# LivGen/LMAT

Hardware: AMD Instinct MI355X
Metric: reads/s (150 bp) vs 64 GB k-mer DB (higher is better)
Workload: dtype u64; 1 GPU; 1104000000 x 150 bp reads/GPU vs 64 GiB k-mer hash (6467472668 20-mers, replicated per GPU), run_rl.sh flags -x 0 -j 30 -l 0 -b 1, calls-only; total_reads=1104000000, reads_per_launch=8000000, read_len=150, db_kmers=6467472668, k=20, parallelism=reads sharded x1, DB replicated, genus_block_permille=100, prune_g=0, list_replicas=1, distinct_lists=792576, reads_called=1058323347, read_pool_batches=32

## Files before the change

### lmat_amd/csrc/kernels.hip

```cpp
#include <hip/hip_runtime.h>
#include <atomic>
#include <type_traits>
#include "kernels.hpp"

#ifndef LMAT_ABLATE
#define LMAT_ABLATE 0
#endif
#define STOP_AT(n, v) do { if (LMAT_ABLATE && A.prm.stop_after == (n)) { if (lane == 0) { emit(250, (v)); } return; } } while (0)
#ifndef LMAT_CLOSURE_FAST
#define LMAT_CLOSURE_FAST 1
#endif
#ifndef LMAT_LIST_INLINE
#define LMAT_LIST_INLINE 1
#endif
#ifndef LMAT_EVEN_K
#define LMAT_EVEN_K 3
#endif
#ifndef LMAT_LDS_SHIFT
#define LMAT_LDS_SHIFT 0
#endif

namespace lmat {

#define WSYNC()                                              \
    do {                                                     \
        __builtin_amdgcn_fence(__ATOMIC_SEQ_CST, "wavefront"); \
        __builtin_amdgcn_wave_barrier();                     \
    } while (0)

template <bool GMEM>
__device__ __forceinline__ void wsync() {
    if (GMEM) __builtin_amdgcn_fence(__ATOMIC_SEQ_CST, "workgroup");
    else __builtin_amdgcn_fence(__ATOMIC_SEQ_CST, "wavefront");
    __builtin_amdgcn_wave_barrier();
}
static const int kGmemU = 32768;
static const int kGmemGrid = 2048;

#define GAS __attribute__((address_space(1)))
typedef uint32_t u32x4 __attribute__((ext_vector_type(4)));
typedef uint32_t u32x4_a4 __attribute__((ext_vector_type(4), aligned(4)));
typedef unsigned short u16x2 __attribute__((ext_vector_type(2)));
typedef uint32_t u32x2 __attribute__((ext_vector_type(2)));
#define LAS __attribute__((address_space(3)))
#define G_ADD(p, v) __hip_atomic_fetch_add((p), (v), __ATOMIC_RELAXED, __HIP_MEMORY_SCOPE_AGENT)
#define G_OR(p, v) __hip_atomic_fetch_or((p), (v), __ATOMIC_RELAXED, __HIP_MEMORY_SCOPE_AGENT)
__device__ __forceinline__ void store_result(GAS uint64_t* dst, const lmat_read_result& r) {
    static_assert(sizeof(lmat_read_result) == 40, "result record is 5 x 8 bytes");
    uint64_t w[5];
    __builtin_memcpy(w, &r, 40);
    dst[0] = w[0]; dst[1] = w[1]; dst[2] = w[2]; dst[3] = w[3]; dst[4] = w[4];
}

__device__ __forceinline__ uint64_t lt_mask(int lane) { return lane == 0 ? 0ull : (~0ull >> (64 - lane)); }
__device__ __forceinline__ int popc64(uint64_t x) { return __popcll(x); }
__device__ __forceinline__ uint32_t wave_scan_incl(uint32_t x) {
    x += (uint32_t)__builtin_amdgcn_update_dpp(0, (int)x, 0x111, 0xf, 0xf, true);
    x += (uint32_t)__builtin_amdgcn_update_dpp(0, (int)x, 0x112, 0xf, 0xf, true);
    x += (uint32_t)__builtin_amdgcn_update_dpp(0, (int)x, 0x114, 0xf, 0xf, true);
    x += (uint32_t)__builtin_amdgcn_update_dpp(0, (int)x, 0x118, 0xf, 0xf, true);
    x += (uint32_t)__builtin_amdgcn_update_dpp(0, (int)x, 0x142, 0xa, 0xf, false);
    x += (uint32_t)__builtin_amdgcn_update_dpp(0, (int)x, 0x143, 0xc, 0xf, false);
    return x;
}
__device__ __forceinline__ uint32_t wave_scan_max(uint32_t x) {
    x = max(x, (uint32_t)__builtin_amdgcn_update_dpp(0, (int)x, 0x111, 0xf, 0xf, true));
    x = max(x, (uint32_t)__builtin_amdgcn_update_dpp(0, (int)x, 0x112, 0xf, 0xf, true));
    x = max(x, (uint32_t)__builtin_amdgcn_update_dpp(0, (int)x, 0x114, 0xf, 0xf, true));
    x = max(x, (uint32_t)__builtin_amdgcn_update_dpp(0, (int)x, 0x118, 0xf, 0xf, true));
    x = max(x, (uint32_t)__builtin_amdgcn_update_dpp(0, (int)x, 0x142, 0xa, 0xf, false));
    x = max(x, (uint32_t)__builtin_amdgcn_update_dpp(0, (int)x, 0x143, 0xc, 0xf, false));
    return x;
}
__device__ __forceinline__ uint32_t wave_sum(uint32_t x) { return (uint32_t)__builtin_amdgcn_readlane((int)wave_scan_incl(x), 63); }
__device__ __forceinline__ uint32_t prefix_count(uint64_t m) {
    return __builtin_amdgcn_mbcnt_hi((uint32_t)(m >> 32), __builtin_amdgcn_mbcnt_lo((uint32_t)m, 0u));
}
__device__ __forceinline__ bool lane_bit(uint64_t m) { return __builtin_amdgcn_inverse_ballot_w64(m); }
__device__ __forceinline__ uint32_t hash32(uint64_t x) {
    x *= 0x9E3779B97F4A7C15ull;
    return (uint32_t)(x >> 40);
}

__device__ __forceinline__ uint32_t zero_bytes(uint32_t z) {
    const uint32_t t = (z & 0x7F7F7F7Fu) + 0x7F7F7F7Fu;
    return ~(t | z | 0x7F7F7F7Fu);
}
__global__ __launch_bounds__(256) void pack_reads_kernel(const uint8_t* __restrict__ bases,
                                                         const uint64_t* __restrict__ off,
                                                         const uint64_t* __restrict__ rec_off,
                                                         uint32_t* __restrict__ words, uint64_t n) {
    const int lane = threadIdx.x & 63;
    const uint32_t sub = (uint32_t)lane & 15u;
    const uint64_t wave = (uint64_t)blockIdx.x * (blockDim.x >> 6) + (threadIdx.x >> 6);
    const uint64_t nw = (uint64_t)gridDim.x * (blockDim.x >> 6);
    for (uint64_t r0 = wave * 4; r0 < n; r0 += nw * 4) {
        const uint64_t r = r0 + ((uint32_t)lane >> 4);
        const bool have = r < n;
        const uint64_t b0 = have ? off[r] : 0;
        const uint32_t len = have ? (uint32_t)(off[r + 1] - b0) : 0u;
        uint32_t* rec = words + (have ? rec_off[r] : 0);
        if (have && sub == 0) rec[0] = len;
        const uint32_t nb = (len + 15) / 16;
        for (uint32_t p0 = 0; __ballot(p0 < len) != 0; p0 += 256) {
            const uint32_t p = p0 + 16u * sub;
            uint32_t code = 0, valid16 = 0;
            if (p < len) {
                const uint64_t addr = b0 + p, a4 = addr & ~3ull, end = b0 + len;
                const uint32_t sh = (uint32_t)(addr & 3) * 8u;
                const uint32_t* src = (const uint32_t*)(bases + a4);
                uint32_t d[5];
#pragma unroll
                for (int q = 0; q < 5; ++q) d[q] = a4 + 4u * q < end ? src[q] : 0u;
                const uint32_t left = len - p;
#pragma unroll
                for (int q = 0; q < 4; ++q) {
                    uint32_t w = __builtin_amdgcn_alignbit(d[q + 1], d[q], sh);
                    if (left < 4u * q + 4u) w &= left > 4u * q ? (1u << (8u * (left - 4u * q))) - 1u : 0u;
                    const uint32_t x = w & 0xDFDFDFDFu;
                    const uint32_t vm = zero_bytes(x ^ 0x41414141u) | zero_bytes(x ^ 0x43434343u) | zero_bytes(x ^ 0x47474747u) | zero_bytes(x ^ 0x54545454u);
                    const uint32_t v1 = vm >> 7;
                    const uint32_t c2 = (((x >> 1) & 0x03030303u) ^ ((x >> 2) & 0x01010101u)) & (v1 * 3u);
                    code |= ((c2 | (c2 >> 6) | (c2 >> 12) | (c2 >> 18)) & 0xFFu) << (8 * q);
                    valid16 |= ((v1 | (v1 >> 7) | (v1 >> 14) | (v1 >> 21)) & 0xFu) << (4 * q);
                }
                if ((p >> 4) < nb) rec[1 + (p >> 4)] = code;
            }
            const uint32_t other = (uint32_t)__shfl_xor((int)valid16, 1);
            if (p < len && (sub & 1u) == 0) rec[1 + nb + (p >> 5)] = valid16 | (other << 16);
        }
    }
}

__device__ __forceinline__ bool wide_insert(uint64_t* slots, uint32_t nbuckets, uint32_t b, uint64_t kmer, uint32_t payload) {
    const uint64_t val = (kmer << kPayloadBits) | payload;
    const uint32_t max_tries = nbuckets < (1u << 14) ? nbuckets : (1u << 14);
    for (uint32_t tries = 0; tries < max_tries; ++tries) {
        unsigned long long* s = (unsigned long long*)(slots + (uint64_t)b * kSlotsPerBucket);
        for (int j = 0; j < kSlotsPerBucket; ++j) {
            unsigned long long old = s[j];
            while (true) {
                if (old == 0) {
                    unsigned long long prev = atomicCAS(&s[j], 0ull, (unsigned long long)val);
                    if (prev == 0) return true;
                    old = prev;
                    continue;
                }
                if ((old >> kPayloadBits) == kmer) {
                    if (old <= val) return true;
                    unsigned long long prev = atomicCAS(&s[j], old, (unsigned long long)val);
                    if (prev == old) return true;
                    old = prev;
                    continue;
                }
                break;
            }
        }
        b = b + 1 == nbuckets ? 0 : b + 1;
    }
    return false;
}
__device__ __forceinline__ uint32_t wide_lookup(const uint64_t* __restrict__ slots, uint32_t nbuckets, uint32_t b, uint64_t kmer) {
    for (uint32_t tries = 0; tries < nbuckets; ++tries) {
        const uint64_t* s = slots + (uint64_t)b * kSlotsPerBucket;
        bool empty = false;
        for (int j = 0; j < kSlotsPerBucket; ++j) {
            const uint64_t v = s[j];
            if (v == 0) empty = true;
            else if ((v >> kPayloadBits) == kmer) return (uint32_t)(v & kPayloadMask);
// ... 221 lines not shown
        const uint32_t nb = (len + 15) / 16;
        for (uint32_t w0 = 0; w0 < nb; w0 += 64) {
            const uint32_t w = w0 + lane;
            uint32_t code = 0, valid = 0;
            if (w < nb) {
                for (int j = 0; j < 16; ++j) {
                    const uint32_t p = w * 16 + j;
                    if (p >= len) break;
                    uint32_t b;
                    if (kind < 10) {
                        b = (uint32_t)(splitmix(h0 ^ ((uint64_t)p << 20) ^ 0x1234567) >> 9) & 3u;
                    } else if (kind == 10) {
                        b = (uint32_t)(splitmix(h0 ^ ((uint64_t)(p % 25) << 20) ^ 0x7654321) >> 9) & 3u;
                    } else {
                        const uint64_t gp = rc ? goff + (len - 1 - p) : goff + p;
                        b = synth_strain_base(g, sp, sg, gp < G ? gp : G - 1);
                        if (rc) b ^= 3u;
                        const uint64_t e = splitmix(h0 ^ ((uint64_t)p << 24) ^ 0xABCDEF);
                        if ((e % 100) == 0) b = (b + 1 + (uint32_t)((e >> 32) % 3)) & 3u;
                    }
                    bool ok = !(kind == 11 && p == npos);
                    code |= (ok ? b : 0u) << (2 * j);
                    valid |= (ok ? 1u : 0u) << j;
                }
                rec[1 + w] = code;
            }
            uint32_t other = __shfl_down(valid, 1);
            if (w < nb && (w & 1) == 0) rec[1 + nb + (w >> 1)] = valid | (((w + 1 < nb) ? other : 0u) << 16);
        }
    }
}

__global__ void lookup_kernel(DeviceTables tb, const uint64_t* __restrict__ kmers, uint64_t n, uint32_t* counts,
                              uint32_t* tids, uint32_t stride) {
    uint64_t i = (uint64_t)blockIdx.x * blockDim.x + threadIdx.x;
    if (i >= n) return;
    const uint32_t pay = table_lookup(tb, kmers[i]);
    if (pay == 0) { counts[i] = 0; return; }
    if (pay < kListBase) {
        counts[i] = 1;
        if (stride) tids[i * stride] = tb.tid32[pay];
        return;
    }
    const size_t eoff = LMAT_LIST_OFF(pay, tb.list_shift);
    if (tb.arena[eoff] & 0x8000u) {
        const uint32_t n = tb.arena[eoff + 1];
        counts[i] = n;
        for (uint32_t j = 0; j < n && j < stride; ++j)
            tids[i * stride + j] = (uint32_t)tb.arena[eoff + kListHdr + 2 * j] | ((uint32_t)tb.arena[eoff + kListHdr + 2 * j + 1] << 16);
        return;
    }
    const uint32_t nk = tb.arena[eoff + 1], nr = tb.arena[eoff + 2];
    counts[i] = nr;
    if (tb.wide) {
        const size_t raw = eoff + kListHdr + 4 * (size_t)nk;
        for (uint32_t j = 0; j < nr && j < stride; ++j) tids[i * stride + j] = (uint32_t)tb.arena[raw + 2 * j] | ((uint32_t)tb.arena[raw + 2 * j + 1] << 16);
        return;
    }
    for (uint32_t j = 0; j < nr && j < stride; ++j) tids[i * stride + j] = tb.conv[tb.arena[eoff + kListHdr + 2 * nk + j]];
}

__global__ void probe_stats_kernel(DeviceTables tb, const uint64_t* __restrict__ kmers, uint64_t n, unsigned long long* out) {
    const uint64_t i = (uint64_t)blockIdx.x * blockDim.x + threadIdx.x;
    if (i >= n || !tb.cpt.nb) return;
    const uint64_t kmer = kmers[i], rc = revcomp_fwd(kmer, tb.cpt.k);
    uint32_t b, tag;
    cpt_address(tb.cpt, kmer < rc ? kmer : rc, kmer < rc ? rc : kmer, b, tag);
    const uint32_t* bk = (const uint32_t*)tb.slots + (uint64_t)b * 16;
    if (kmer <= rc)
        for (int j = 0; j < kCptSlots; ++j)
            if (((const uint16_t*)bk)[j] == (uint16_t)tag) { atomicAdd(&out[0], 1ull); return; }
    if (!(bk[15] & kCptOvfFlag)) { atomicAdd(&out[1], 1ull); return; }
    uint32_t ob = ovf_bucket_of(b, tag, tb.ovf_nbuckets);
    unsigned long long reads = 0;
    for (uint32_t tries = 0; tries < tb.ovf_nbuckets; ++tries) {
        const uint64_t* s_ = tb.ovf_slots + (uint64_t)ob * kSlotsPerBucket;
        ++reads;
        bool empty = false;
        for (int j = 0; j < kSlotsPerBucket; ++j) {
            const uint64_t v = s_[j];
            if (v == 0) empty = true;
            else if ((v >> kPayloadBits) == kmer) { atomicAdd(&out[2], 1ull); atomicAdd(&out[4], reads); return; }
        }
        if (empty) break;
        ob = ob + 1 == tb.ovf_nbuckets ? 0 : ob + 1;
    }
    atomicAdd(&out[3], 1ull);
    atomicAdd(&out[4], reads);
}

struct LinEnt {
    uint16_t tid;
    uint16_t dep;
    uint16_t tin, tout;
    float score;
};
static const uint16_t kLinNoGood = 0x8000;
struct LinEntW {
    uint32_t tid;
    uint16_t dep, pad_;
    uint32_t tin, tout;
    float score;
};
static const int kFastE = 256;
static const int kK4SmallT = 16;
static const int kK4MidT = 32;
template <int TT> struct K4Lds {
    static constexpr int LIN = TT + (TT <= 16 ? 3 : 8);
    static constexpr int LANES = TT <= 32 ? 64 : 32;
    static constexpr int STRIDE = ((17 * TT + 12 * LIN + 3) / 4) | 1;
    static constexpr int BYTES = STRIDE * 4 * LANES;
    static_assert(8 * TT <= 12 * LIN, "sort keys over the lineage entries");
};
static_assert(K4Lds<16>::STRIDE == 125, "small tier: 31.25 KB per wave");

constexpr int pow2_ceil(int x) { int p = 1; while (p < x) p <<= 1; return p; }

template <int U, int T, int E, bool INK4, bool CPT = false, bool WIDE = false>
struct WL {
    static constexpr int IDB = WIDE ? 4 : 2;
    static constexpr int HB = WIDE ? 8 : 4;
    static_assert(!WIDE || INK4, "wide ids run in the classes that keep their tables in memory and decide in-kernel");
    static constexpr int H = pow2_ceil(U * 3 / 2);
    static constexpr int D = INK4 ? U : 64;
    static constexpr int TH = 4 * T;
    static constexpr int LIN = T + 72;
    static constexpr int RD_WORDS = (U + 96) / 16 + (U + 96) / 32 + 4;
    static constexpr int R1_HASH = 8 * H;
    static constexpr int R1_TID = (IDB + 6) * T + 2 * HB * TH + (INK4 ? (4 + 2 * IDB) * T + 4 * T + T + 4 * T + 4 * T + T : 0);
    static constexpr bool HASH_OVER = CPT && U <= 512 && !INK4;
    static constexpr int R1 = HASH_OVER ? R1_TID : (R1_HASH > R1_TID ? R1_HASH : R1_TID);
    static constexpr int R2_K = CPT ? 0 : 8 * U + 4 * U;
    static constexpr int R2_D = 4 * D + 2 * D + 2 * D + 2 * D + D;
    static constexpr int R2_L = INK4 ? (WIDE ? 20 : 12) * LIN : 0;
    static constexpr int R2 = R2_K > R2_D ? (R2_K > R2_L ? R2_K : R2_L) : (R2_D > R2_L ? R2_D : R2_L);
    static constexpr int R3_P = 4 * U;
    static constexpr int R3_E = (INK4 ? (WIDE ? 24 : 16) : 7) * E;
    static constexpr int R3 = R3_P > R3_E ? R3_P : R3_E;
    static constexpr int OFF_RD = 0;
    static constexpr int OFF_R1 = CPT && U <= 512 ? 0 : ((RD_WORDS * 4 + 15) / 16) * 16;
    static constexpr int OFF_R2 = OFF_R1 + ((R1 + 15) / 16) * 16;
    static constexpr int OFF_R3 = OFF_R2 + ((R2 + 15) / 16) * 16;
    static constexpr int BYTES_BASE = OFF_R3 + ((R3 + 15) / 16) * 16;
    static constexpr int XL_STAGE = 2048, XL_GBKT = XL_STAGE, XL_BLOOM = XL_GBKT + 256, XL_OLIST = XL_BLOOM + 512;
    static constexpr int XL_BYTES = XL_OLIST + 1024;
    static_assert(!(CPT && U <= 512) || RD_WORDS * 4 <= XL_STAGE, "the record lies under the stage, which K1 does not touch");
    static constexpr bool XL_OVERLAY = U <= 512;
    static constexpr int OFF_XL = XL_OVERLAY ? OFF_R1 : BYTES_BASE;
    static constexpr int OFF_UPAY_C = XL_OVERLAY && OFF_R1 + XL_BYTES > OFF_R3 ? OFF_R1 + XL_BYTES : OFF_R3;
    static constexpr int BYTES_C = XL_OVERLAY ? (OFF_UPAY_C + 4 * U > BYTES_BASE ? ((OFF_UPAY_C + 4 * U + 15) / 16) * 16 : BYTES_BASE)
                                              : BYTES_BASE + XL_BYTES;
    static constexpr int BYTES_H = HASH_OVER && OFF_R1 + R1_HASH > BYTES_C ? OFF_R1 + R1_HASH : BYTES_C;
    static constexpr int BYTES = CPT ? BYTES_H : BYTES_BASE;
};

static const uint64_t kEmpty64 = ~0ull;

__device__ __forceinline__ uint32_t lds_min_insert(unsigned long long* hv, int hmask, uint64_t key, uint32_t idx) {
    const unsigned long long v = (key << 16) | idx;
    uint32_t h = hash32(key) & hmask;
    while (true) {
        unsigned long long old = hv[h];
        if (old == kEmpty64 || (old >> 16) == key) {
            if (old != kEmpty64 && old <= v) return h;
            unsigned long long prev = atomicCAS(&hv[h], old, v);
            if (prev == old) return h;
        } else {
            h = (h + 1) & hmask;
        }
    }
}
__device__ __forceinline__ uint32_t lds_find(const unsigned long long* hv, int hmask, uint64_t key) {
    uint32_t h = hash32(key) & hmask;
    while ((hv[h] >> 16) != key) h = (h + 1) & hmask;
    return h;
}

__device__ __forceinline__ uint32_t tid_hash(uint32_t t, int thmask) { return (__umul24(t, 0x9E3779u) >> 10) & thmask; }
__device__ __forceinline__ uint32_t tid_find_or_claim(unsigned int* hent, int thmask, uint32_t t) {
    uint32_t h = tid_hash(t, thmask);
    while (true) {
        unsigned int cur = hent[h];
        if ((cur & 0xFFFFu) == t) return h;
        if (cur == 0) {
            unsigned int prev = atomicCAS(&hent[h], 0u, t | 0xFFFF0000u);
            if (prev == 0 || (prev & 0xFFFFu) == t) return h;
        }
        h = (h + 1) & thmask;
    }
}
__device__ __forceinline__ int tid_find(const unsigned int* hent, int thmask, uint32_t t) {
    uint32_t h = tid_hash(t, thmask);
    while (true) {
        unsigned int cur = hent[h];
        if ((cur & 0xFFFFu) == t) return (int)h;
        if (cur == 0) return -1;
        h = (h + 1) & thmask;
    }
}
__device__ __forceinline__ int tid_slot(const unsigned int* hent, int thmask, uint32_t t) {
    const int h = tid_find(hent, thmask, t);
    if (h < 0) return -1;
    const uint32_t s = hent[h] >> 16;
    return s >= 0x8000u ? -1 : (int)s;
}
__device__ __forceinline__ uint32_t tid_hash_w(uint32_t t, int thmask) { return ((t * 0x9E3779B1u) >> 12) & thmask; }
__device__ __forceinline__ uint32_t tid_find_or_claim(unsigned long long* hent, int thmask, uint32_t t) {
    uint32_t h = tid_hash_w(t, thmask);
    while (true) {
        unsigned long long cur = hent[h];
        if ((uint32_t)cur == t) return h;
        if (cur == 0) {
            unsigned long long prev = atomicCAS(&hent[h], 0ull, (unsigned long long)t | 0xFFFFFFFF00000000ull);
            if (prev == 0 || (uint32_t)prev == t) return h;
        }
        h = (h + 1) & thmask;
    }
}
__device__ __forceinline__ int tid_find(const unsigned long long* hent, int thmask, uint32_t t) {
    uint32_t h = tid_hash_w(t, thmask);
    while (true) {
        unsigned long long cur = hent[h];
        if ((uint32_t)cur == t) return (int)h;
        if (cur == 0) return -1;
        h = (h + 1) & thmask;
    }
}
__device__ __forceinline__ int tid_slot(const unsigned long long* hent, int thmask, uint32_t t) {
    const int h = tid_find(hent, thmask, t);
    if (h < 0) return -1;
    const uint32_t s = (uint32_t)(hent[h] >> 32);
    return s >= 0x80000000u ? -1 : (int)s;
}
__device__ __forceinline__ void add_u16(uint16_t* arr, uint32_t idx, uint32_t v) {
    atomicAdd((unsigned int*)arr + (idx >> 1), (idx & 1) ? (v << 16) : v);
}

__device__ __forceinline__ bool anc_iv(uint32_t tin_a, uint32_t tout_a, uint32_t tin_b, uint32_t tout_b) {
    return tin_a < tin_b && tout_b <= tout_a;
}

struct K4Key { uint32_t lo, hi; };
struct TCmpDev {
    const float* score;
    const uint16_t* dep;
    __device__ bool operator()(uint16_t a, uint16_t b) const {
        const float d = score[a] - score[b];
        if ((double)fabsf(d) < 0.001) return (int)dep[a] < (int)dep[b];
        return score[a] < score[b];
    }
};
struct CmpDepthDev {
    template <class LE> __device__ bool operator()(const LE& a, const LE& b) const { return (int)(a.dep & 0x7FFF) > (int)(b.dep & 0x7FFF); }
};

__device__ __constant__ double kLogfInvC[16] = {
    0x1.661ec79f8f3bep+0, 0x1.571ed4aaf883dp+0, 0x1.49539f0f010bp+0, 0x1.3c995b0b80385p+0, 0x1.30d190c8864a5p+0,
    0x1.25e227b0b8eap+0, 0x1.1bb4a4a1a343fp+0, 0x1.12358f08ae5bap+0, 0x1.0953f419900a7p+0, 0x1p+0,
    0x1.e608cfd9a47acp-1, 0x1.ca4b31f026aap-1, 0x1.b2036576afce6p-1, 0x1.9c2d163a1aa2dp-1, 0x1.886e6037841edp-1,
    0x1.767dcf5534862p-1};
__device__ __constant__ double kLogfLogC[16] = {
    -0x1.57bf7808caadep-2, -0x1.2bef0a7c06ddbp-2, -0x1.01eae7f513a67p-2, -0x1.b31d8a68224e9p-3, -0x1.6574f0ac07758p-3,
    -0x1.1aa2bc79c81p-3, -0x1.a4e76ce8c0e5ep-4, -0x1.1973c5a611cccp-4, -0x1.252f438e10c1ep-5, 0x0p+0,
    0x1.aa5aa5df25984p-5, 0x1.c5e53aa362eb4p-4, 0x1.526e57720db08p-3, 0x1.bc2860d22477p-3, 0x1.1058bc8a07ee1p-2,
    0x1.4043057b6ee09p-2};
__device__ __forceinline__ float glibc_logf(float x) {
    uint32_t ix = __float_as_uint(x);
    if (ix == 0x3f800000u) return 0.0f;
    if (ix - 0x00800000u >= 0x7f800000u - 0x00800000u) {
        if (ix * 2 == 0) return -__builtin_inff();
        if (ix == 0x7f800000u) return x;
        if ((ix & 0x80000000u) || ix * 2 >= 0xff000000u) return __builtin_nanf("");
        ix = __float_as_uint(x * 0x1p23f);
        ix -= 23u << 23;
    }
    const uint32_t tmp = ix - 0x3f330000u;
    const int i = (tmp >> (23 - 4)) % 16;
    const int k = (int32_t)tmp >> 23;
    const uint32_t iz = ix - (tmp & 0xff800000u);
    const double invc = kLogfInvC[i], logc = kLogfLogC[i];
    const double z = (double)__uint_as_float(iz);
    const double r = z * invc - 1.0;
    const double y0 = logc + (double)k * 0x1.62e42fefa39efp-1;
    const double r2 = r * r;
    double y = 0x1.5575b0be00b6ap-2 * r + -0x1.ffffef20a4123p-2;
    y = -0x1.00ea348b88334p-2 * r2 + y;
    y = y * r2 + (y0 + r);
    return (float)y;
}

__device__ __forceinline__ int nm_table_of(const NullModelDev& nm, uint32_t cand) {
    if (!nm.active) return -1;
    const GAS int* len_vec = (const GAS int*)nm.len_vec;
    const GAS int* len_avg = (const GAS int*)nm.len_avg;
    const GAS int* len_table = (const GAS int*)nm.len_table;
    int i = 0;
    for (; i < nm.n_len - 1; ++i)
        if ((int)cand <= len_avg[i]) break;
    const int len = len_vec[i];
    return len > 0 ? len_table[i] : len_table[nm.n_len];
}

struct K4State {
    float top_score, diff_thresh;
    int lidx, nlin, lowest, highest;
    unsigned highest_depth;
// ... 1440 lines not shown
                if ((uint32_t)lane < lpr) te = ((const GAS u32x4*)A.tail16)[ri * lpr + lane];
                if (lane < 3) tu = ((const GAS uint64_t*)A.tail_u)[ri * 4 + lane];
                kreg[c] = ((uint64_t)(te.y & 0xFFu) << 32) | te.x;
                hreg[c] = te.z;
                treg[c] = te.w & 0xC0000000u;
                okm[c] = __ballot((te.w >> 24) & 1u);
                valid_kmers += popc64(okm[c]);
                ureg[c] = tu;
                if (128u + (uint32_t)lane < P) upay[128 + lane] = te.w & 0xFFFFFFu;
                continue;
            }
            pass1_chunk((uint32_t)c * 64, kreg[c], hreg[c], treg[c], okm[c], ureg[c], fcm[c]);
        }
        STOP_AT(47, 0);
        if (CPT) {
            if constexpr (LSH) {
                WSYNC();
                LAS uint64_t* ush = (LAS uint64_t*)xl;
#pragma unroll
                for (int c = 0; c < CH; ++c) ush[c * 64 + lane] = ureg[c];
                if (lane < 4) ush[CH * 64 + lane] = 0ull;
                WSYNC();
            }
#pragma unroll
            for (int c = 0; c < CH; ++c) {
                if (!UNI && (uint32_t)c * 64 >= P) break;
                if (TAILOK && c == 2 && tail_mode()) continue;
                cpt_finish(c, kreg[c], ureg[c], c + 1 < CH ? ureg[c + 1] : 0ull, fcm[c], hreg[c], treg[c]);
            }
        }
    } else {
        for (uint32_t p0 = 0; p0 < len; p0 += 64) { uint64_t a; uint32_t b, t; uint64_t v, u, f; pass1_chunk(p0, a, b, t, v, u, f); }
    }
    WSYNC();
    if (tot > 0) {
        const float q = (float)gc / (float)tot;
        const float gc_pcnt = (float)((double)q * 100.0);
        bin_sel = __builtin_amdgcn_readfirstlane((int)(gc_pcnt / 10.0f));
    }
    if (valid_kmers < A.prm.min_kmer) {
        if (lane == 0) { emit(LMAT_ST_SHORT_VALID, 0); nmacc[0]++; }
        return;
    }
    STOP_AT(1, 0);
    RELANE();
    uint32_t nuniq = 0;
    uint32_t nscan = 0;
    if constexpr (!CPT) {
    auto pass2_chunk = [&](uint32_t p0, uint64_t km, uint32_t h, bool ok) {
        const uint32_t p = p0 + lane;
        const bool first = ok && (uint32_t)(hv[h] & 0xFFFF) == p;
        const uint64_t bm = __ballot(first);
        if (first) {
            const uint32_t rk = nuniq + prefix_count(bm);
            ukmer[rk] = (km << kPayloadBits) + 1;
            ubucket[rk] = bucket_of(km, tb.nbuckets);
            upay[rk] = 0;
        }
        nuniq += popc64(bm);
    };
    if (CACHE) {
#pragma unroll
        for (int c = 0; c < CH; ++c) {
            if (!UNI && (uint32_t)c * 64 >= P) break;
            pass2_chunk((uint32_t)c * 64, kreg[c], hreg[c], lane_bit(okm[c]));
        }
    } else {
        for (uint32_t p0 = 0; p0 < P; p0 += 64) {
            const uint32_t p = p0 + lane;
            uint64_t km = 0, kr = 0;
            uint32_t h = 0;
            bool fc;
            const bool ok = p < P && window(p, km, kr, fc);
            if (ok) h = lds_find(hv, L::H - 1, km);
            pass2_chunk(p0, km, h, ok);
        }
    }
    WSYNC();
    nscan = nuniq;
    if (!PLAIN && A.prm.stop_after == 2) { if (lane == 0) { emit(250, nuniq); } return; }
    RELANE();
    {
        const GAS u32x4* quarters = (const GAS u32x4*)g_slots;
        uint16_t* plist = (uint16_t*)hv;
        uint32_t npend = 0;
        auto probe = [&](auto nb_tag, auto nl_tag, auto ident_tag, uint32_t np, const uint16_t* pcur, uint16_t* pnext) {
            constexpr int NB = decltype(nb_tag)::value;
            constexpr int NLX = decltype(nl_tag)::value;
            constexpr bool IDENT = decltype(ident_tag)::value;
            constexpr int LPK = 4 * NB;
            constexpr int KPL = 64 / LPK;
            constexpr uint32_t GM = NB == 4 ? 0xFFFFu : (NB == 2 ? 0xFFu : 0xFu);
            const int gk = lane / LPK, bi = (lane >> 2) & (NB - 1), q4 = lane & 3;
            for (uint32_t base = 0; base < np; base += NLX * KPL) {
                u32x4 sl[NLX];
#pragma unroll
                for (int i = 0; i < NLX; ++i) {
                    const uint32_t li = base + i * KPL + gk;
                    u32x4 v = {0u, 0u, 0u, 0u};
                    if (li < np) {
                        uint32_t b = ubucket[IDENT ? li : (uint32_t)pcur[li]] + bi;
                        if (b >= tb.nbuckets) b -= tb.nbuckets;
                        v = quarters[(uint64_t)b * 4 + q4];
                    }
                    sl[i] = v;
                }
#pragma unroll
                for (int i = 0; i < NLX; ++i) {
                    if (base + i * KPL >= np) break;
                    const uint32_t li = base + i * KPL + gk;
                    const bool act = li < np;
                    const uint32_t idx = act ? (IDENT ? li : (uint32_t)pcur[li]) : 0u;
                    const uint64_t kmsh1 = act ? ukmer[idx] : 0ull;
                    const uint64_t t0 = (((uint64_t)sl[i].y << 32) | sl[i].x) - kmsh1;
                    const uint64_t t1 = (((uint64_t)sl[i].w << 32) | sl[i].z) - kmsh1;
                    const bool m0 = act && t0 < 0xFFFFFFull, m1 = act && t1 < 0xFFFFFFull;
                    const bool free_slot = act && q4 == 3 && (sl[i].z | sl[i].w) == 0u;
                    const uint32_t se = (uint32_t)(__ballot(m0 || m1 || free_slot) >> (gk * LPK)) & GM;
                    const int settle = se ? (__builtin_ctz(se) >> 2) : NB;
                    if ((m0 || m1) && bi == settle) upay[idx] = (uint32_t)(m0 ? t0 : t1) + 1u;
                    const bool pend = act && (lane & (LPK - 1)) == 0 && settle == NB;
                    const uint64_t pm = __ballot(pend);
                    if (pend) {
                        uint32_t b = ubucket[idx] + NB;
                        if (b >= tb.nbuckets) b -= tb.nbuckets;
                        ubucket[idx] = b;
                        pnext[npend + prefix_count(pm)] = (uint16_t)idx;
                    }
                    npend += (uint32_t)popc64(pm);
                }
            }
        };
        constexpr int NL = (U + 15) / 16 < 9 ? (U + 15) / 16 : 9;
        probe(std::integral_constant<int, 1>{}, std::integral_constant<int, NL>{}, std::true_type{}, nuniq, plist, plist + U);
        WSYNC();
        int round = 1;
        while (npend > 0) {
            const uint16_t* pcur = plist + ((round & 1) ? U : 0);
            uint16_t* pnext = plist + ((round & 1) ? 0 : U);
            const uint32_t np = npend;
            npend = 0;
            if (round == 1) probe(std::integral_constant<int, 2>{}, std::integral_constant<int, 5>{}, std::false_type{}, np, pcur, pnext);
            else probe(std::integral_constant<int, 4>{}, std::integral_constant<int, 2>{}, std::false_type{}, np, pcur, pnext);
            WSYNC();
            ++round;
        }
    }
    WSYNC();
    } else {
    LAS uint32_t* stage = (LAS uint32_t*)xl;
    LAS uint32_t* gbkt = (LAS uint32_t*)(xl + L::XL_GBKT);
    LAS unsigned int* bloomA = (LAS unsigned int*)(xl + L::XL_BLOOM);
    LAS unsigned int* bloomB = (LAS unsigned int*)(xl + L::XL_BLOOM + 256);
    LAS u32x4* olist = (LAS u32x4*)(xl + L::XL_OLIST);
    const GAS u32x4* quarters = (const GAS u32x4*)g_slots;
    uint64_t firstm[KC];
    bool suspect = !CACHE;
    if (CACHE) {
        constexpr bool DIG = !EVENK;
        constexpr uint32_t kNone = 0xFFFFFFFFu;
        uint32_t pb = 0, pq = kNone, ps1 = kNone, ps2 = kNone, ps3 = kNone;
        uint64_t seen = 0;
        LAS uint32_t* barr = (LAS uint32_t*)xl;
        LAS uint32_t* sarr = barr + (64 * CH + 4);
        LAS uint16_t* qarr = (LAS uint16_t*)(sarr + (64 * CH + 4));
        if constexpr (LSH) {
            static_assert(10 * (64 * CH + 4) <= WL<U, T, E, INK4, CPT>::XL_BLOOM, "the parked values end below the repeat filter's bits");
            WSYNC();
            if (lane < 3) { barr[lane] = 0u; if (DIG) sarr[lane] = kNone; qarr[lane] = 0xFFFF; }
#pragma unroll
            for (int c = 0; c < CH; ++c) {
                if (!UNI && (uint32_t)c * 64 >= P) break;
                barr[3 + c * 64 + lane] = hreg[c];
                if (DIG) sarr[3 + c * 64 + lane] = lane_bit(okm[c]) ? (uint32_t)(kreg[c] ^ (kreg[c] >> 17)) : kNone;
                qarr[3 + c * 64 + lane] = lane_bit(okm[c]) ? (uint16_t)((uint32_t)c * 64 + lane + (treg[c] >> 30)) : (uint16_t)0xFFFF;
            }
            WSYNC();
        }
#pragma unroll
        for (int c = 0; c < CH; ++c) {
            if (!UNI && (uint32_t)c * 64 >= P) break;
            const uint64_t V = okm[c];
            const uint32_t b = hreg[c];
            const uint32_t sig = DIG && lane_bit(V) ? (uint32_t)(kreg[c] ^ (kreg[c] >> 17)) : kNone;
            const uint32_t q = lane_bit(V) ? (uint32_t)c * 64 + lane + (treg[c] >> 30) : (LSH ? 0xFFFFu : kNone);
            uint32_t bprev, qprev, s1 = 0, s2 = 0, s3 = 0;
            if constexpr (LSH) {
                bprev = barr[c * 64 + lane + 2];
                qprev = qarr[c * 64 + lane + 2];
                if constexpr (DIG) { s1 = sarr[c * 64 + lane + 2]; s2 = sarr[c * 64 + lane + 1]; s3 = sarr[c * 64 + lane]; }
            } else {
                bprev = (uint32_t)__builtin_amdgcn_update_dpp((int)pb, (int)b, 0x138, 0xf, 0xf, false);
                qprev = (uint32_t)__builtin_amdgcn_update_dpp((int)pq, (int)q, 0x138, 0xf, 0xf, false);
                if constexpr (DIG) {
                    s1 = (uint32_t)__builtin_amdgcn_update_dpp((int)ps1, (int)sig, 0x138, 0xf, 0xf, false);
                    s2 = (uint32_t)__builtin_amdgcn_update_dpp((int)ps2, (int)s1, 0x138, 0xf, 0xf, false);
                    s3 = (uint32_t)__builtin_amdgcn_update_dpp((int)ps3, (int)s2, 0x138, 0xf, 0xf, false);
                }
            }
            uint64_t hitm = 0;
            if constexpr (DIG) hitm = V & (__ballot(sig == s1) | __ballot(sig == s2) | __ballot(sig == s3));
            const uint64_t openm = V & ~(__ballot(b == bprev) & __ballot(q == qprev));
            uint32_t both = 0;
            if (lane_bit(openm)) {
                const uint32_t h1 = b & 2047u, h2 = (b >> 11) & 2047u;
                const unsigned int oa = __hip_atomic_fetch_or(&bloomA[h1 >> 5], 1u << (h1 & 31), __ATOMIC_RELAXED, __HIP_MEMORY_SCOPE_WORKGROUP);
                const unsigned int ob = __hip_atomic_fetch_or(&bloomB[h2 >> 5], 1u << (h2 & 31), __ATOMIC_RELAXED, __HIP_MEMORY_SCOPE_WORKGROUP);
                both = (oa >> (h1 & 31)) & (ob >> (h2 & 31)) & 1u;
            }
            hitm |= __ballot(both != 0u);
            seen |= hitm;
            if constexpr (!LSH) {
                pb = (uint32_t)__builtin_amdgcn_readlane((int)b, 63);
                pq = (uint32_t)__builtin_amdgcn_readlane((int)q, 63);
                if constexpr (DIG) {
                    ps1 = (uint32_t)__builtin_amdgcn_readlane((int)sig, 63);
                    ps2 = (uint32_t)__builtin_amdgcn_readlane((int)sig, 62);
                    ps3 = (uint32_t)__builtin_amdgcn_readlane((int)sig, 61);
                }
            }
        }
        suspect = seen != 0;
    }
    if (suspect) {
        for (int i = lane; i < L::H; i += 64) hv[i] = kEmpty64;
        WSYNC();
        if (CACHE) {
#pragma unroll
            for (int c = 0; c < CH; ++c) {
                if (!UNI && (uint32_t)c * 64 >= P) break;
                const bool ok = lane_bit(okm[c]);
                uint32_t h = 0;
                if (ok) h = lds_min_insert(hv, L::H - 1, kreg[c], (uint32_t)c * 64 + lane);
                treg[c] = (treg[c] & 0xC000FFFFu) | (h << 16);
            }
            WSYNC();
#pragma unroll
            for (int c = 0; c < CH; ++c) {
                if (!UNI && (uint32_t)c * 64 >= P) break;
                const bool ok = lane_bit(okm[c]);
                firstm[c] = __ballot(ok && (uint32_t)(hv[(treg[c] >> 16) & 0x3FFFu] & 0xFFFF) == (uint32_t)c * 64 + lane);
                nuniq += popc64(firstm[c]);
            }
        } else {
            for (uint32_t p0 = 0; p0 < P; p0 += 64) {
                const uint32_t p = p0 + lane;
                uint64_t km = 0, kr = 0;
                bool fc;
                if (p < P && window(p, km, kr, fc)) lds_min_insert(hv, L::H - 1, km, p);
            }
        }
        WSYNC();
    } else {
#pragma unroll
        for (int c = 0; c < CH; ++c) {
            if (!UNI && (uint32_t)c * 64 >= P) break;
            firstm[c] = okm[c];
            nuniq += popc64(okm[c]);
        }
    }
    STOP_AT(46, nuniq);
    RELANE();
    uint32_t nov = 0;
    auto ovf_pass = [&]() {
      constexpr int OVL = (!INK4 && E <= kFastE && U <= 256) ? (U <= 160 ? 2 : 1) : 3;
      const GAS u32x4* oq = (const GAS u32x4*)tb.ovf_slots;
      const int q4 = lane & 3;
      for (uint32_t e0 = 0; e0 < nov; e0 += 16 * OVL) {
        u32x4 v[OVL];
        uint32_t ob[OVL];
#pragma unroll
        for (int g = 0; g < OVL; ++g) {
            const uint32_t en = e0 + 16u * g + ((uint32_t)lane >> 2);
            v[g] = u32x4{1u, 0u, 1u, 0u};
            ob[g] = 0;
            if (en < nov) {
                const u32x4 e = olist[en];
                ob[g] = ovf_bucket_of(e.z, e.w & 0xFFFFu, tb.ovf_nbuckets);
                v[g] = oq[(uint64_t)ob[g] * 4 + q4];
            }
        }
#pragma unroll
        for (int g = 0; g < OVL; ++g) {
            if (e0 + 16u * g >= nov) break;
            const uint32_t en = e0 + 16u * g + ((uint32_t)lane >> 2);
            bool act = en < nov;
            u32x4 e = {0u, 0u, 0u, 0u};
            if (act) e = olist[en];
            const uint64_t key1 = ((((uint64_t)e.y << 32) | e.x) << kPayloadBits) + 1;
            u32x4 vv = v[g];
            uint32_t obg = ob[g];
            while (true) {
                const uint64_t t0 = (((uint64_t)vv.y << 32) | vv.x) - key1, t1 = (((uint64_t)vv.w << 32) | vv.z) - key1;
                const bool m0 = act && t0 < 0xFFFFFFull, m1 = act && t1 < 0xFFFFFFull;
                if (m0 || m1) upay[e.w >> 16] = (uint32_t)(m0 ? t0 : t1) + 1u;
                const uint32_t done = (uint32_t)(__ballot(m0 || m1 || (q4 == 3 && (vv.z | vv.w) == 0u)) >> (lane & ~3)) & 0xFu;
                if (done) act = false;
                if (!__ballot(act)) break;
                obg = obg + 1 == tb.ovf_nbuckets ? 0 : obg + 1;
                vv = u32x4{1u, 0u, 1u, 0u};
                if (act) vv = oq[(uint64_t)obg * 4 + q4];
            }
        }
      }
      nov = 0;
    };
    auto probe_chunk = [&](uint32_t p0, uint64_t km, uint32_t b, uint32_t tag, uint64_t okmask, uint64_t firstmask) {
        const uint32_t p = p0 + lane;
        const uint64_t V1 = okmask << 1;
        const uint32_t bprev = (uint32_t)__builtin_amdgcn_update_dpp(0, (int)b, 0x138, 0xf, 0xf, false);
        const uint64_t lm = okmask & ~(V1 & __ballot(b == bprev));
        const bool leader = lane_bit(lm);
        const uint32_t ng = (uint32_t)popc64(lm);
        const uint32_t gidx = prefix_count(lm) + (leader ? 1u : 0u) - 1u;
        if (leader) gbkt[gidx] = b;
        WSYNC();
        uint32_t pay = 0;
        uint32_t spillw = 0;
        for (uint32_t g0 = 0; g0 < ng; g0 += 32) {
#pragma unroll
            for (int s = 0; s < 2; ++s) {
                if (g0 + (uint32_t)s * 16 < ng) {
                    const uint32_t g = g0 + (uint32_t)s * 16 + ((uint32_t)lane >> 2);
                    if (g < ng) {
                        const uint32_t gb = gbkt[g];
                        __builtin_amdgcn_global_load_lds((const GAS void*)(quarters + (uint64_t)gb * 4 + (lane & 3)),
                                                         (LAS void*)(xl + s * 1024), 16, 0, 0);
                    }
                }
            }
            __builtin_amdgcn_s_waitcnt(0);
            WSYNC();
            if (lane_bit(okmask & __ballot(gidx - g0 < 32u))) {
                const LAS uint32_t* bk = stage + (gidx - g0) * 16;
                const u32x4 t0 = *(const LAS u32x4*)bk;
                const uint32_t t4 = bk[4], t5 = bk[5];
                const uint32_t key2 = tag | (tag << 16);
                auto z = [&](uint32_t x) -> uint32_t {
                    uint32_t r;
                    asm("v_pk_min_u16 %0, %1, %2" : "=v"(r) : "v"(x ^ key2), "v"(0x00010001u));
                    return r;
                };
                const uint32_t miss = z(t0.x) | (z(t0.y) << 1) | (z(t0.z) << 2) | (z(t0.w) << 3) | (z(t4) << 4) | (z(t5) << 5);
                const uint32_t acc = ~miss & 0x003F003Fu;
                if (acc) {
                    const uint32_t bit = (uint32_t)__builtin_ctz(acc);
                    const uint32_t slot = 2 * (bit & 15u) + (bit >> 4);
                    pay = (uint32_t)((const LAS uint16_t*)bk)[12 + slot] | ((uint32_t)((const LAS uint8_t*)bk)[48 + slot] << 16);
                } else {
                    spillw = bk[15];
                }
            }
            if (g0 + 32 < ng) WSYNC();
        }
        static_assert(kCptOvfFlag == 0x80000000u, "the spill flag is the sign bit");
        if (UNI || p < P) upay[p] = lane_bit(firstmask) ? pay : 0u;
        const uint64_t pm = firstmask & __ballot((int32_t)spillw < 0);
        if (pm) {
            if (nov + (uint32_t)popc64(pm) > 64u) { WSYNC(); ovf_pass(); WSYNC(); }
            if (lane_bit(pm)) olist[nov + prefix_count(pm)] = u32x4{(uint32_t)km, (uint32_t)(km >> 32), b, tag | (p << 16)};
            nov += (uint32_t)popc64(pm);
        }
        WSYNC();
    };
    if (CACHE) {
#pragma unroll
        for (int c = 0; c < CH; ++c) {
            if (!UNI && (uint32_t)c * 64 >= P) break;
            if (TAILOK && c == 2 && tail_mode()) {
                if (suspect && 128u + (uint32_t)lane < P && !lane_bit(firstm[c])) upay[128 + lane] = 0u;
                WSYNC();
                continue;
            }
            probe_chunk((uint32_t)c * 64, kreg[c], hreg[c], treg[c] & 0xFFFFu, okm[c], firstm[c]);
        }
    } else {
        for (uint32_t p0 = 0; p0 < P; p0 += 64) {
            const uint32_t p = p0 + lane;
            uint64_t km = 0, kr = 0;
            uint32_t b = 0, t = 0;
            bool fc;
            const bool ok = p < P && window(p, km, kr, fc);
            bool first = false;
            if (ok) {
                cpt_address(*(const CptGeom*)&tb.cpt, km, kr, b, t);
                first = (uint32_t)(hv[lds_find(hv, L::H - 1, km)] & 0xFFFF) == p;
            }
            const uint64_t fm = __ballot(first);
            nuniq += (uint32_t)popc64(fm);
            probe_chunk(p0, km, b, t, __ballot(ok), fm);
        }
    }
    if (nov) { ovf_pass(); WSYNC(); }
    nscan = P;
    if (!PLAIN && A.prm.stop_after == 2) { if (lane == 0) { emit(250, nuniq); } return; }
    }
    STOP_AT(3, upay[0]);
    RELANE();
    uint32_t ndist = 0;
    bool many = false;
    if constexpr (U <= 320) {
        constexpr int KP = (U + 63) / 64;
        uint32_t pv[KP];
        uint64_t rm[KP];
#pragma unroll
        for (int c = 0; c < KP; ++c) {
            const uint32_t i = (uint32_t)c * 64 + lane;
            pv[c] = i < nscan ? upay[i] : 0u;
            rm[c] = __ballot(pv[c] != 0u);
        }
        uint32_t dp_reg = 0, dm_reg = 0;
#pragma unroll
        for (int c0 = 0; c0 < KP; ++c0) {
            while (rm[c0]) {
                const uint32_t v = (uint32_t)__builtin_amdgcn_readlane((int)pv[c0], __builtin_ctzll(rm[c0]));
                uint32_t cn = 0;
#pragma unroll
                for (int c = c0; c < KP; ++c) {
                    const uint64_t m = __ballot(pv[c] == v);
                    cn += (uint32_t)popc64(m);
                    rm[c] &= ~m;
                }
                uint32_t m0_keep;
                asm volatile("s_mov_b32 %2, m0\n\ts_mov_b32 m0, %4\n\tv_writelane_b32 %0, %3, m0\n\tv_writelane_b32 %1, %5, m0\n\ts_mov_b32 m0, %2"
                             : "+v"(dp_reg), "+v"(dm_reg), "=&s"(m0_keep) : "s"(v), "s"(ndist), "s"(cn));
                ++ndist;
            }
        }
        many = ndist > 64u;
        if (!many) {
            if ((uint32_t)lane < ndist) { dpay[lane] = dp_reg; dmult[lane] = (uint16_t)dm_reg; }
            WSYNC();
        }
    } else {
        uint32_t dp_reg = 0, dm_reg = 0;
        for (uint32_t i0 = 0; i0 < nscan && !many; i0 += 64) {
            const uint32_t i = i0 + lane;
            const uint32_t pay = i < nscan ? upay[i] : 0;
            uint64_t rem = __ballot(pay != 0);
            while (rem) {
                const uint32_t v = (uint32_t)__builtin_amdgcn_readlane((int)pay, __builtin_ctzll(rem));
                const uint64_t m = __ballot(pay == v);
                const uint32_t c = (uint32_t)popc64(m);
                const uint64_t ex = __ballot((uint32_t)lane < ndist && dp_reg == v);
                if (ex) {
                    if (lane == __builtin_ctzll(ex)) dm_reg += c;
                } else {
                    if (ndist >= 64) { many = true; break; }
                    if ((uint32_t)lane == ndist) { dp_reg = v; dm_reg = c; }
                    ++ndist;
                }
                rem &= ~m;
            }
        }
        if (!many) {
            if ((uint32_t)lane < ndist) { dpay[lane] = dp_reg; dmult[lane] = (uint16_t)dm_reg; }
            WSYNC();
        }
    }
    if (many && !INK4) {
        if (lane == 0) {
            emit(255, 0);
            if (A.ovf_list) ((GAS uint32_t*)A.ovf_list)[G_ADD(&g_cursor[A.ovf_slot], 1u)] = (uint32_t)r;
            else G_OR(g_err, (uint32_t)kErrTidOverflow);
        }
        return;
    }
    if (INK4 && many) {
        for (int i = lane; i < L::H; i += 64) hv[i] = kEmpty64;
        WSYNC();
        for (uint32_t i0 = 0; i0 < nscan; i0 += 64) {
            const uint32_t i = i0 + lane;
            const uint32_t pay = i < nscan ? upay[i] : 0;
            if (pay) lds_min_insert(hv, L::H - 1, pay, i);
        }
        WSYNC();
        ndist = 0;
        for (uint32_t i0 = 0; i0 < nscan; i0 += 64) {
            const uint32_t i = i0 + lane;
            const uint32_t pay = i < nscan ? upay[i] : 0;
            bool owner = false;
            uint32_t h = 0;
            if (pay) {
                h = lds_find(hv, L::H - 1, pay);
                owner = (uint32_t)(hv[h] & 0xFFFF) == i;
            }
            const uint64_t bm = __ballot(owner);
            WSYNC();
            if (owner) {
                const uint32_t rk = ndist + prefix_count(bm);
                dpay[rk] = pay;
                hv[h] = ((unsigned long long)pay << 16) | (0x8000u | rk);
            }
            ndist += popc64(bm);
        }
        for (uint32_t d = lane; d < (ndist + 1) / 2; d += 64) ((unsigned int*)dmult)[d] = 0;
        WSYNC();
        for (uint32_t i0 = 0; i0 < nscan; i0 += 64) {
            const uint32_t i = i0 + lane;
            const uint32_t pay = i < nscan ? upay[i] : 0;
            if (pay) add_u16(dmult, (uint32_t)(hv[lds_find(hv, L::H - 1, pay)] & 0x7FFFu), 1u);
        }
        WSYNC();
    }
    if (!PLAIN && A.prm.stop_after == 4) { if (lane == 0) { emit(250, ndist); } return; }
    if (ndist == 0) {
        if (lane == 0) { emit(LMAT_ST_NODBHITS, 0); nmacc[1]++; }
        return;
    }
    RELANE();
    if (!PLAIN && A.gene_mode) {
        uint32_t* gkey = (uint32_t*)hent;
        uint32_t* gval = (uint32_t*)best;
        uint32_t* greg = (uint32_t*)reg;
        uint32_t* gcnt = (uint32_t*)cnt;
        uint16_t* gord = (uint16_t*)(lds + L::OFF_R3);
        const GAS uint16_t* arena = g_arena;
        uint32_t nel = 0;
        bool overflow = false;
        for (uint32_t d0 = 0; d0 < ndist; d0 += 64) {
// ... 1564 lines not shown
```

Baseline: 446.4 million reads/s.

## Merge first two chunk probes into one batched bucket gather via larger LDS stage

For the 160-position CPT class, the first two 64-k-mer chunks are now probed together. Their distinct bucket leaders go into one group list, and up to four wave-loads of buckets are gathered into a bigger LDS stage with global_load_lds, followed by a single wait. The overflow list moves into the idle R3 region and gains a capacity-aware add routine. The aim is to raise memory-level parallelism and cut per-chunk sync and wait rounds, at the cost of tighter LDS overlay constraints and more complex code.

Measured after the change: 450.8 million reads/s (median of 2 runs). Within noise of the previous version (+1.0%).

```diff
diff --git a/lmat_amd/csrc/kernels.hip b/lmat_amd/csrc/kernels.hip
--- a/lmat_amd/csrc/kernels.hip
+++ b/lmat_amd/csrc/kernels.hip
@@ -15,6 +15,9 @@
 #endif
 #ifndef LMAT_EVEN_K
 #define LMAT_EVEN_K 3
+#endif
+#ifndef LMAT_PROBE_MERGED
+#define LMAT_PROBE_MERGED 1
 #endif
 #ifndef LMAT_LDS_SHIFT
 #define LMAT_LDS_SHIFT 0
@@ -542,6 +545,18 @@
                                               : BYTES_BASE + XL_BYTES;
     static constexpr int BYTES_H = HASH_OVER && OFF_R1 + R1_HASH > BYTES_C ? OFF_R1 + R1_HASH : BYTES_C;
     static constexpr int BYTES = CPT ? BYTES_H : BYTES_BASE;
+    static constexpr bool XL_MERGED = LMAT_PROBE_MERGED && CPT && U == 160 && !INK4;
+    static constexpr int XL_STAGE_M = XL_BYTES, XL_STAGE_CAP_M = XL_STAGE_M / 64;
+    static constexpr int XL_GBKT_M = XL_STAGE_M - 4 * 128;
+    static_assert(!XL_MERGED || XL_GBKT_M >= 3 * 1024, "the first three wave-loads leave the group buckets alone");
+    static constexpr int XL_OLIST_M = OFF_UPAY_C - OFF_XL + 4 * U;
+    static constexpr int XL_OLIST_ROOM_M = (BYTES_C - OFF_XL - XL_OLIST_M) / 16;
+    static constexpr int XL_OLIST_CAP_M = XL_OLIST_ROOM_M < 64 ? XL_OLIST_ROOM_M : 64;
+    static_assert(!XL_MERGED || (XL_OVERLAY && OFF_XL == OFF_R1), "the merged probe's block overlays the tables");
+    static_assert(!XL_MERGED || OFF_XL + XL_STAGE_M <= OFF_UPAY_C, "the stage ends below upay");
+    static_assert(!XL_MERGED || (XL_OLIST_M % 16 == 0 && XL_OLIST_M >= XL_STAGE_M), "the list is aligned and lies behind the stage");
+    static_assert(!XL_MERGED || (XL_OLIST_CAP_M >= 32 && OFF_XL + XL_OLIST_M + 16 * XL_OLIST_CAP_M <= BYTES_C), "the list fits behind upay");
+    static_assert(!XL_MERGED || OFF_XL + XL_OLIST_M >= OFF_R3, "the list lies in R3, idle until K3");
 };
 
 static const uint64_t kEmpty64 = ~0ull;
@@ -2288,7 +2303,9 @@
     LAS uint32_t* gbkt = (LAS uint32_t*)(xl + L::XL_GBKT);
     LAS unsigned int* bloomA = (LAS unsigned int*)(xl + L::XL_BLOOM);
     LAS unsigned int* bloomB = (LAS unsigned int*)(xl + L::XL_BLOOM + 256);
-    LAS u32x4* olist = (LAS u32x4*)(xl + L::XL_OLIST);
+    constexpr bool MERGED = L::XL_MERGED && (LMAT_PROBE_MERGED == 1 || PLAIN);
+    static_assert(!MERGED || (CACHE && CH == 3), "the merged probe is for the classes of three chunks whose k-mers stay in registers");
+    LAS u32x4* olist = (LAS u32x4*)(xl + (MERGED ? L::XL_OLIST_M : L::XL_OLIST));
     const GAS u32x4* quarters = (const GAS u32x4*)g_slots;
     uint64_t firstm[KC];
     bool suspect = !CACHE;
@@ -2440,6 +2457,16 @@
         }
       }
       nov = 0;
+    };
+    auto olist_add = [&](uint64_t pm, uint64_t km, uint32_t b, uint32_t tag, uint32_t p) {
+        while (pm) {
+            const uint32_t rank = prefix_count(pm);
+            const uint64_t take = pm & __ballot(rank < (uint32_t)L::XL_OLIST_CAP_M - nov);
+            if (lane_bit(take)) olist[nov + rank] = u32x4{(uint32_t)km, (uint32_t)(km >> 32), b, tag | (p << 16)};
+            nov += (uint32_t)popc64(take);
+            pm &= ~take;
+            if (pm) { WSYNC(); ovf_pass(); WSYNC(); }
+        }
     };
     auto probe_chunk = [&](uint32_t p0, uint64_t km, uint32_t b, uint32_t tag, uint64_t okmask, uint64_t firstmask) {
         const uint32_t p = p0 + lane;
@@ -2492,16 +2519,104 @@
         static_assert(kCptOvfFlag == 0x80000000u, "the spill flag is the sign bit");
         if (UNI || p < P) upay[p] = lane_bit(firstmask) ? pay : 0u;
         const uint64_t pm = firstmask & __ballot((int32_t)spillw < 0);
-        if (pm) {
+        if constexpr (MERGED) olist_add(pm, km, b, tag, p);
+        else if (pm) {
             if (nov + (uint32_t)popc64(pm) > 64u) { WSYNC(); ovf_pass(); WSYNC(); }
             if (lane_bit(pm)) olist[nov + prefix_count(pm)] = u32x4{(uint32_t)km, (uint32_t)(km >> 32), b, tag | (p << 16)};
             nov += (uint32_t)popc64(pm);
         }
         WSYNC();
     };
+    auto probe_pair = [&]() {
+      if constexpr (MERGED) {
+        constexpr uint32_t CAP = (uint32_t)L::XL_STAGE_CAP_M;
+        static_assert(CAP > 48 && CAP <= 64, "four wave-loads of 16 buckets, the last one partly");
+        LAS uint32_t* gbkt = (LAS uint32_t*)(xl + L::XL_GBKT_M);
+        auto leaders = [&](int c) -> uint64_t {
+            const uint32_t bprev = (uint32_t)__builtin_amdgcn_update_dpp(0, (int)hreg[c], 0x138, 0xf, 0xf, false);
+            return okm[c] & ~((okm[c] << 1) & __ballot(hreg[c] == bprev));
+        };
+        uint32_t gidx[2];
+        uint32_t ngt = 0;
+#pragma unroll
+        for (int c = 0; c < 2; ++c) {
+            const uint64_t lm = leaders(c);
+            gidx[c] = ngt + prefix_count(lm) + (lane_bit(lm) ? 1u : 0u) - 1u;
+            asm volatile("" : "+v"(gidx[c]));
+            ngt += (uint32_t)popc64(lm);
+            if (lane_bit(lm) && gidx[c] < CAP) gbkt[gidx[c]] = hreg[c];
+        }
+        for (uint32_t g0 = 0;;) {
+            if (g0) {
+#pragma unroll
+                for (int c = 0; c < 2; ++c) {
+                    if (lane_bit(leaders(c)) && gidx[c] - g0 < CAP) gbkt[gidx[c] - g0] = hreg[c];
+                }
+            }
+            WSYNC();
+            const uint32_t n = ngt - g0 < CAP ? ngt - g0 : CAP;
+            uint32_t lg = (uint32_t)lane >> 2;
+            asm volatile("" : "+v"(lg));
+            uint32_t gb3 = 0;
+            if (48u + lg < n) gb3 = gbkt[48u + lg];
+            asm volatile("" : "+v"(gb3));
+#pragma unroll
+            for (int s = 0; s < 3; ++s) {
+                if ((uint32_t)s * 16 < n) {
+                    const uint32_t g = (uint32_t)s * 16 + lg;
+                    if (g < n) {
+                        const uint32_t gb = gbkt[g];
+                        __builtin_amdgcn_global_load_lds((const GAS void*)(quarters + (uint64_t)gb * 4 + (lane & 3)),
+                                                         (LAS void*)(xl + s * 1024), 16, 0, 0);
+                    }
+                }
+            }
+            asm volatile("" ::: "memory");
+            if (48u + lg < n) {
+                __builtin_amdgcn_global_load_lds((const GAS void*)(quarters + (uint64_t)gb3 * 4 + (lane & 3)), (LAS void*)(xl + 3 * 1024), 16, 0, 0);
+            }
+            __builtin_amdgcn_s_waitcnt(0);
+            WSYNC();
+#pragma unroll
+            for (int c = 0; c < 2; ++c) {
+                const uint32_t p = (uint32_t)c * 64 + lane;
+                const uint32_t tag = treg[c] & 0xFFFFu;
+                const uint64_t inr = okm[c] & __ballot(gidx[c] - g0 < CAP);
+                uint32_t pay = 0, spillw = 0;
+                if (lane_bit(inr)) {
+                    const LAS uint32_t* bk = stage + (gidx[c] - g0) * 16;
+                    const u32x4 t0 = *(const LAS u32x4*)bk;
+                    const uint32_t t4 = bk[4], t5 = bk[5];
+                    const uint32_t key2 = tag | (tag << 16);
+                    auto z = [&](uint32_t x) -> uint32_t {
+                        uint32_t r;
+                        asm("v_pk_min_u16 %0, %1, %2" : "=v"(r) : "v"(x ^ key2), "v"(0x00010001u));
+                        return r;
+                    };
+                    const uint32_t miss = z(t0.x) | (z(t0.y) << 1) | (z(t0.z) << 2) | (z(t0.w) << 3) | (z(t4) << 4) | (z(t5) << 5);
+                    const uint32_t acc = ~miss & 0x003F003Fu;
+                    if (acc) {
+                        const uint32_t bit = (uint32_t)__builtin_ctz(acc);
+                        const uint32_t slot = 2 * (bit & 15u) + (bit >> 4);
+                        pay = (uint32_t)((const LAS uint16_t*)bk)[12 + slot] | ((uint32_t)((const LAS uint8_t*)bk)[48 + slot] << 16);
+                    } else {
+                        spillw = bk[15];
+                    }
+                }
+                const uint64_t wr = g0 == 0 ? inr | ~okm[c] : inr;
+                if (lane_bit(wr) && (UNI || p < P)) upay[p] = lane_bit(firstm[c]) ? pay : 0u;
+                olist_add(firstm[c] & inr & __ballot((int32_t)spillw < 0), kreg[c], hreg[c], tag, p);
+            }
+            g0 += CAP;
+            WSYNC();
+            if (g0 >= ngt) break;
+        }
+      }
+    };
     if (CACHE) {
-#pragma unroll
-        for (int c = 0; c < CH; ++c) {
+        if constexpr (MERGED) probe_pair();
+#pragma unroll
+        for (int c = MERGED ? 2 : 0; c < CH; ++c) {
             if (!UNI && (uint32_t)c * 64 >= P) break;
             if (TAILOK && c == 2 && tail_mode()) {
                 if (suspect && 128u + (uint32_t)lane < P && !lane_bit(firstm[c])) upay[128 + lane] = 0u;
```
